# retrojetpacks/Gadget-Leicester

Hardware: AMD Instinct MI355X
Metric: particle-steps/sec (gravity+SPH) (higher is better)
Workload: dtype f64

## Files before the change

### gadget-leicester_amd/csrc/ghip_gravity.hip

```cpp
#include <cmath>

#include "ghip_prim.h"
#include "ghip_walk.h"

__global__ void k_grav_finish(int nt, const int *__restrict__ tgt, const int *__restrict__ perm,
                              int n, double G, double comoving_fac, const double *__restrict__ pos,
                              const double *__restrict__ gravpm, double *__restrict__ oacc,
                              double *__restrict__ oldacc)
{
  int ti = blockIdx.x * blockDim.x + threadIdx.x;
  if(ti >= nt)
    return;
  int i = perm[tgt[ti]];
  double a0 = oacc[i], a1 = oacc[(size_t) n + i], a2 = oacc[2 * (size_t) n + i];
  if(comoving_fac != 0)
    {
      a0 += comoving_fac * pos[i];
      a1 += comoving_fac * pos[(size_t) n + i];
      a2 += comoving_fac * pos[2 * (size_t) n + i];
    }
  double b0 = a0, b1 = a1, b2 = a2;
  if(gravpm)
    {
      b0 = a0 + gravpm[i] / G;
// ... 298 lines not shown
  k_build_segments<<<cdiv(total, 64), 64, 0, ctx->stream>>>(
    ts, P<int4>(t.lk), T, P<int>(t.seg_start), P<int>(t.seg_nanc), P<int>(t.seg_anc));
  HIPCHK(hipGetLastError());
  if(!walk_records)
    return GHIP_OK;
  return ghip_fill_walk_records(ctx, t);
}

int ghip_fill_walk_records(ghip_ctx *ctx, TreeDev &t)
{
  const TreeSizes *ts = P<TreeSizes>(t.dsz);
  const long long ce = (long long) t.n + t.cap_nodes;
  if(ce + 2 >= (1LL << 26))
    return ghip_fail(ctx, GHIP_EINVAL, "the walk addresses its 64-byte element records by a 32-bit byte "
                     "offset: room for %lld elements is more than 2^26", ce);
  GCHK(ghip_ensure(ctx, t.mq, (size_t) (ce + 1) * sizeof(WalkHot)));
  GCHK(ghip_ensure(ctx, t.mq2, (size_t) (ce + 1) * sizeof(WalkCold)));
  k_fill_elems<<<cdiv(ce, 256), 256, 0, ctx->stream>>>(ts, P<double4>(t.xm), P<double4>(t.cl),
                                                      P<int4>(t.lk), P<double>(t.aux),
                                                      P<WalkHot>(t.mq), P<WalkCold>(t.mq2));
  HIPCHK(hipGetLastError());
  return GHIP_OK;
}

int ghip_walk_layout(const TreeDev &t, WalkSeg &sg, int table)
{
  sg.ns = t.seg_ns[table];
  sg.nsub = sg.ns < GHIP_MAXSUB ? sg.ns : GHIP_MAXSUB;
  if(getenv("GHIP_WALK_SUBS"))
    {
      int v = atoi(getenv("GHIP_WALK_SUBS"));
      if(v >= 1 && v <= sg.ns)
        sg.nsub = v;
    }
  if(sg.nsub < 1)
    sg.nsub = 1;
  sg.start = P<int>(t.seg_start) + t.seg_soff[table];
  sg.nanc = P<int>(t.seg_nanc) + t.seg_noff[table];
  sg.anc = P<int>(t.seg_anc) + (size_t) t.seg_noff[table] * GHIP_MAXANC;
  return sg.nsub;
}

static int walk_layout(const TreeDev &t, int nt, WalkSeg &sg, int *nbuckets, bool ewald)
{
  *nbuckets = (nt + 63) / 64;
  static int mid_min = -1;
  if(mid_min < 0)
    {
      mid_min = 3072;
      if(getenv("GHIP_WALK_MID_MIN"))
        mid_min = atoi(getenv("GHIP_WALK_MID_MIN"));
    }
  int table = ewald ? (*nbuckets >= mid_min ? 2 : 1) : (*nbuckets >= mid_min ? 1 : 0);
  return ghip_walk_layout(t, sg, table);
}

struct PartialBufs
{
  double *ax, *ay, *az;
  int *cost;
};

static int ensure_partials(ghip_ctx *ctx, int nwaves, int slot, PartialBufs &pb)
{
  size_t cnt = (size_t) nwaves * 64;
  DevBuf &bx = slot ? ctx->tax2 : ctx->tax, &by = slot ? ctx->tay2 : ctx->tay,
         &bz = slot ? ctx->taz2 : ctx->taz, &bc = slot ? ctx->tcost2 : ctx->tcost;
  GCHK(ghip_ensure(ctx, bx, cnt * 8));
  GCHK(ghip_ensure(ctx, by, cnt * 8));
  GCHK(ghip_ensure(ctx, bz, cnt * 8));
  GCHK(ghip_ensure(ctx, bc, cnt * 4));
  pb.ax = P<double>(bx);
  pb.ay = P<double>(by);
  pb.az = P<double>(bz);
  pb.cost = P<int>(bc);
  return GHIP_OK;
}

static int build_plan(ghip_ctx *ctx, int kind, int nb, int ns, WalkPlan &plan, int slot = 0,
                      hipStream_t on = nullptr)
{
  hipStream_t st = on ? on : ctx->stream;
  DevBuf &b_nsub = slot ? ctx->plan_nsub2 : ctx->plan_nsub, &b_woff = slot ? ctx->plan_woff2 : ctx->plan_woff,
         &b_wave = slot ? ctx->plan_wave2 : ctx->plan_wave;
  int sbase = (49152 + nb - 1) / nb;
  sbase = sbase < 8 ? 8 : (sbase > 64 ? 64 : sbase);
  if(sbase > ns)
    sbase = ns;
  if(getenv("GHIP_WALK_SUBS"))
    {
      int v = atoi(getenv("GHIP_WALK_SUBS"));
      if(v >= 1 && v <= ns)
        sbase = v;
    }
  const int maxwaves = (sbase + 2) * nb + 8;
  GCHK(ghip_ensure(ctx, b_nsub, (size_t) nb * 4));
  GCHK(ghip_ensure(ctx, b_woff, (size_t) (nb + 1) * 4));
  GCHK(ghip_ensure(ctx, b_wave, (size_t) maxwaves * 4));
  int cur = ctx->plan_cur[kind];
  bool prev_kept = ctx->plan_steps[kind][cur].p != nullptr;
  const size_t steps_bytes = ((size_t) nb + nb / 8 + 64) * 4;
  for(int k = 0; k < 2; k++)
    if(ctx->plan_steps[kind][k].cap < (size_t) nb * 4)
      {
        GCHK(ghip_ensure(ctx, ctx->plan_steps[kind][k], steps_bytes));
        if(k == cur)
          prev_kept = false;
      }
  const bool adaptive = !(getenv("GHIP_WALK_ADAPTIVE") && atoi(getenv("GHIP_WALK_ADAPTIVE")) == 0);
  const int pnb = ctx->plan_nb[kind];
  int tol = nb / 16 < 8 ? 8 : nb / 16;
  if(getenv("GHIP_PLAN_EXACT") && atoi(getenv("GHIP_PLAN_EXACT")))
    tol = ctx->plan_ns[kind] == ns ? 0 : -1;
  bool have_prev = adaptive && kind < 2 && pnb > 0 && (pnb > nb ? pnb - nb : nb - pnb) <= tol && prev_kept;
  int nprev = have_prev ? (pnb < nb ? pnb : nb) : 0;
  if(getenv("GHIP_PLAN_DEBUG") && kind < 2)
    {
      static int calls[2], used[2];
      calls[kind]++;
      used[kind] += have_prev;
      if(calls[kind] % 16 == 0)
        fprintf(stderr, "ghip plan kind %d: history used in %d of %d calls (nb %d, before %d)\n", kind,
                used[kind], calls[kind], nb, pnb);
    }
  unsigned int *prev = P<unsigned int>(ctx->plan_steps[kind][cur]);
  unsigned int *out = P<unsigned int>(ctx->plan_steps[kind][cur ^ 1]);
  k_plan_nsub<<<cdiv(nb, 256), 256, 0, st>>>(nb, ns, sbase, prev, nprev, P<int>(b_nsub));
  GCHK(ghip_scan(ctx, P<int>(b_nsub), P<int>(b_woff), nb, st, slot ? &ghip_prim_scratch(ctx, ctx->stream2) : nullptr));
  HIPCHK(hipMemsetAsync(b_wave.p, 0xff, (size_t) maxwaves * 4, st));
  k_plan_fill<<<cdiv(nb, 256), 256, 0, st>>>(nb, P<int>(b_nsub), P<int>(b_woff),
                                             maxwaves, P<int>(b_wave), out,
                                             ghip_errword(ctx, GHIP_ERRW_PLAN));
  HIPCHK(hipGetLastError());
  if(kind < 2)
    {
      ctx->plan_nb[kind] = nb;
      ctx->plan_ns[kind] = ns;
      ctx->plan_cur[kind] = cur ^ 1;
    }
  plan.nwaves = maxwaves;
  plan.wave_bucket = P<int>(b_wave);
  plan.woff = P<int>(b_woff);
  plan.nsub = P<int>(b_nsub);
  plan.steps_out = out;
  plan.started = nullptr;
  plan.started_at = 0;
  return GHIP_OK;
}

template <int MODE>
static void launch_walk(ghip_ctx *ctx, const TreeDev &t, const WalkSeg &sg, int nbuckets, int nt,
                        const int *tgt, const double *tx, const double *ty, const double *tz,
                        const double *tsoft, const double *toldacc, const GravK &k,
                        unsigned long long *counter, const WalkPlan &plan, const PartialBufs &pb,
                        hipStream_t stream)
{
  long long nthreads = (long long) plan.nwaves * 64;
  int bsize = 64;
  if(getenv("GHIP_WALK_BLOCK"))
    {
      int v = atoi(getenv("GHIP_WALK_BLOCK"));
      if(v == 64 || v == 128 || v == 256)
        bsize = v;
    }
  int blocks = cdiv(nthreads, bsize);
  blocks = (blocks + 7) & ~7;
  if(k.xcd_remap > 1)
    blocks = ((blocks + 8 * k.xcd_remap - 1) / (8 * k.xcd_remap)) * (8 * k.xcd_remap);
  WalkPlan pl = plan;
  if(pl.started)
    {
      static double frac = -1;
      if(frac < 0)
        frac = getenv("GHIP_HYDRO_TRIGGER_AT") ? atof(getenv("GHIP_HYDRO_TRIGGER_AT")) : 1.0;
      pl.started_at = (int) (frac * (blocks - 1));
      if(pl.started_at > blocks - 1 || pl.started_at < 0)
        pl.started_at = blocks - 1;
    }
  static int lds_env = -1;
  if(lds_env < 0)
    lds_env = getenv("GHIP_PAIR_NEWTON_LDS") ? atoi(getenv("GHIP_PAIR_NEWTON_LDS")) : 0;
  const int lds_n = lds_env > 0 ? lds_env : ctx->pair_lds;
  static int cap_min = -1;
  if(cap_min < 0)
    cap_min = getenv("GHIP_PAIR_CAP_MIN") ? atoi(getenv("GHIP_PAIR_CAP_MIN")) : 1536;
  static int lds_e = -1;
  if(lds_e < 0)
    lds_e = getenv("GHIP_PAIR_EWALD_LDS") ? atoi(getenv("GHIP_PAIR_EWALD_LDS")) : 0;
  const size_t dyn_lds =
    (MODE == GHIP_WALK_NEWTON && stream != ctx->stream && nbuckets >= cap_min)
      ? (size_t) lds_n
      : ((MODE == GHIP_WALK_EWALD && stream != ctx->stream && nbuckets >= cap_min) ? (size_t) lds_e : 0);
#define GHIP_LAUNCH_WALK(PER, UNEQ)                                                              \
  k_grav_walk<MODE, PER, UNEQ><<<blocks, bsize, dyn_lds, stream>>>(                                \
    t.nelem, P<WalkHot>(t.mq), P<WalkCold>(t.mq2), sg, nt, tgt, tx, ty, tz, tsoft, toldacc, k,     \
    P<float>(ctx->srtab), P<double>((UNEQ) && MODE == GHIP_WALK_EWALD ? ctx->ewbrick : ctx->ewtab),  \
    pb.ax, pb.ay, pb.az, pb.cost, getenv("GHIP_WALK_NOCOUNT") ? nullptr : counter,                  \
    P<unsigned long long>(ctx->rslots) + (counter - P<unsigned long long>(ctx->cslots)), pl)
  static int brick_env = -2;
  if(brick_env == -2)
    brick_env = getenv("GHIP_EW_BRICK") ? atoi(getenv("GHIP_EW_BRICK")) : -1;
  const bool brick = brick_env >= 0 ? brick_env != 0 : true;
  const bool uneq = (MODE == GHIP_WALK_EWALD) ? brick : (bool) k.unequal;
  if(k.periodic && uneq)
    GHIP_LAUNCH_WALK(true, true);
  else if(k.periodic)
    GHIP_LAUNCH_WALK(true, false);
  else if(uneq)
    GHIP_LAUNCH_WALK(false, true);
  else
    GHIP_LAUNCH_WALK(false, false);
#undef GHIP_LAUNCH_WALK
}

static void launch_walk_any(ghip_ctx *ctx, int walk, const TreeDev &t, const WalkSeg &sg,
                            int nbuckets, int nt, const int *tgt, const double *tx,
                            const double *ty, const double *tz, const double *tsoft,
                            const double *toldacc, const GravK &k, unsigned long long *counter,
                            const WalkPlan &plan, const PartialBufs &pb, hipStream_t stream)
{
  if(walk == GHIP_WALK_NEWTON)
    launch_walk<GHIP_WALK_NEWTON>(ctx, t, sg, nbuckets, nt, tgt, tx, ty, tz, tsoft, toldacc, k,
                                  counter, plan, pb, stream);
  else if(walk == GHIP_WALK_SHORTRANGE)
    launch_walk<GHIP_WALK_SHORTRANGE>(ctx, t, sg, nbuckets, nt, tgt, tx, ty, tz, tsoft, toldacc, k,
                                      counter, plan, pb, stream);
  else
    launch_walk<GHIP_WALK_EWALD>(ctx, t, sg, nbuckets, nt, tgt, tx, ty, tz, tsoft, toldacc, k,
                                 counter, plan, pb, stream);
}

static void shard_slice(const ghip_ctx *ctx, int nt, int *lo, int *cnt)
{
  int per;
  ghip_shard_range(nt, ctx->shard_n, ctx->shard_rank, lo, cnt, &per);
}

struct WalkJob
{
  int walk;
  GravK k;
  WalkSeg sg;
  WalkPlan plan;
  PartialBufs pb;
  int nbuckets;
  unsigned long long *counter;
};

static int prepare_job(ghip_ctx *ctx, const ghip_grav_params *p, int walk, int nt, int slot,
                       WalkJob &J, hipStream_t plan_on = nullptr)
{
  hipStream_t ps = plan_on ? plan_on : ctx->stream;
  J.walk = walk;
  GCHK(prepare_tables(ctx, p, walk, J.k));
  walk_layout(ctx->dyn_use ? ctx->dyn.tree : ctx->gt, nt, J.sg, &J.nbuckets, walk == GHIP_WALK_EWALD);
  GCHK(build_plan(ctx, walk == GHIP_WALK_EWALD ? 1 : 0, J.nbuckets, J.sg.ns, J.plan, slot, ps));
  GCHK(ensure_partials(ctx, J.plan.nwaves, slot, J.pb));
  J.counter = ghip_cslot(ctx, walk == GHIP_WALK_EWALD ? GHIP_CK_EWALD : GHIP_CK_NEWTON);
  HIPCHK(hipMemsetAsync(J.counter, 0, GHIP_CKIND_U64 * 8, ps));
  return GHIP_OK;
}

static int run_walk(ghip_ctx *ctx, const WalkJob &J, int nt, const int *tgt, hipStream_t st)
{
  int evi = (J.walk == GHIP_WALK_EWALD) ? 4 : 2;
  ctx->plan_writer[J.walk == GHIP_WALK_EWALD ? 1 : 0] = st;
  HIPCHK(hipEventRecord(ctx->evp[evi], st));
  launch_walk_any(ctx, J.walk, ctx->dyn_use ? ctx->dyn.tree : ctx->gt, J.sg, J.nbuckets, nt, tgt, P<double>(ctx->sx),
                  P<double>(ctx->sy), P<double>(ctx->sz), P<double>(ctx->ssoft),
                  P<double>(ctx->soldacc), J.k, J.counter, J.plan, J.pb, st);
  HIPCHK(hipGetLastError());
  HIPCHK(hipEventRecord(ctx->evp[evi + 1], st));
  return GHIP_OK;
}

static int combine_walk(ghip_ctx *ctx, const WalkJob &J, int nt, const int *tgt, hipStream_t st)
{
  k_combine_grav<<<cdiv(nt, 256), 256, 0, st>>>(
    nt, J.plan, tgt, P<int>(ctx->gt.perm), J.pb.ax, J.pb.ay, J.pb.az, J.pb.cost, ctx->n,
    P<double>(ctx->f[GHIP_F_GRAVACCEL]), P<int>(ctx->f[GHIP_F_GRAVCOST]),
    J.walk == GHIP_WALK_EWALD ? 1 : 0, J.k.debug_steps);
  HIPCHK(hipGetLastError());
  return GHIP_OK;
}

static const int pair_caps[GHIP_PAIR_NSET] = {GHIP_PAIR_LDS(6), GHIP_PAIR_LDS(5), GHIP_PAIR_LDS(4)};

static int pair_setting(int lds)
{
  int k = 0;
  for(int j = 1; j < GHIP_PAIR_NSET; j++)
    if(lds >= pair_caps[j])
      k = j;
  return k;
}

static int pair_balance(ghip_ctx *ctx)
{
  if(!ctx->pc_ev[3][3])
    {
      for(int i = 0; i < 4; i++)
        for(int j = 0; j < 4; j++)
          if(!ctx->pc_ev[i][j])
            HIPCHK(hipEventCreate(&ctx->pc_ev[i][j]));
      return GHIP_OK;
    }
  bool pending[GHIP_PAIR_NSET] = {};
  for(int i = 0; i < 4; i++)
    {
      if(ctx->pc_cap[i] == 0)
        continue;
      hipEvent_t *e = ctx->pc_ev[i];
      if(hipEventQuery(e[1]) != hipSuccess || hipEventQuery(e[3]) != hipSuccess)
        {
          (void) hipGetLastError();
          pending[pair_setting(ctx->pc_cap[i])] = true;
          continue;
        }
      float tn = 0, te = 0;
      if(hipEventElapsedTime(&tn, e[0], e[1]) == hipSuccess && hipEventElapsedTime(&te, e[2], e[3]) == hipSuccess)
        {
          const int k = pair_setting(ctx->pc_cap[i]);
          const float fe = ctx->pc_hyd[i] ? 1.1f : 1.0f;
          const float c = tn > fe * te ? tn : fe * te;
          ctx->pc_cost[k] = c;
          ctx->pc_age[k] = 0;
        }
      else
        (void) hipGetLastError();
      ctx->pc_cap[i] = 0;
    }
  for(int k = 0; k < GHIP_PAIR_NSET; k++)
    ctx->pc_age[k]++;
  const int cur = pair_setting(ctx->pair_lds);
  const float *cost = ctx->pc_cost;
  if(cost[cur] < 0)
    return GHIP_OK;
  int want = cur, probe = -1;
  for(int k = 0; k < GHIP_PAIR_NSET; k++)
// ... 299 lines not shown
```

### gadget-leicester_amd/csrc/ghip_internal.h

```cpp
#pragma once
#include <hip/hip_runtime.h>

#include <cstdint>
#include <cstdio>
#include <cstdlib>
#include <cstring>
#include <new>
#include <string>
#include <vector>

#include "../../include/ghip.h"
#include "ghip_count.h"

#define GHIP_BITS 21
#define GHIP_EN 64
#define GHIP_EW_NB ((GHIP_EN >> 1) + 1)
#define GHIP_EW_NKB (GHIP_EN / 3 + 1)
#define GHIP_EW_DOUBLES (GHIP_EW_NB * GHIP_EW_NB * GHIP_EW_NKB * 16)
static inline __host__ __device__ unsigned int ghip_ew_offset(int i, int j, int kb, int t)
{
  return (unsigned int) ((((i >> 1) * GHIP_EW_NB + (j >> 1)) * GHIP_EW_NKB + kb) * 16 +
                         ((i & 1) * 2 + (j & 1)) * 4 + t);
}
#define GHIP_NTAB 1000
// ... 269 lines not shown
struct PmFft
{
  int n = 0;
  void *fwd = nullptr, *inv = nullptr;
  DevBuf rho, k;
  PmFft() = default;
  PmFft(const PmFft &) = delete;
  PmFft &operator=(const PmFft &) = delete;
  ~PmFft();
};

struct PmMesh
{
  PmFft fft;
  DevBuf force;
  struct Open
  {
    PmFft fft;
    int table_n = 0;
    DevBuf table, force, oct;
  } open;
};

#define GHIP_LDS_PER_CU 163840
#define GHIP_LDS_GRANULE 2048
#define GHIP_PAIR_LDS(W) ((GHIP_LDS_PER_CU / (4 * (W))) / GHIP_LDS_GRANULE * GHIP_LDS_GRANULE)
#define GHIP_PAIR_NSET 3
static_assert(GHIP_PAIR_LDS(4) == 10240 && GHIP_PAIR_LDS(5) == 8192 && GHIP_PAIR_LDS(6) == 6144,
              "dynamic-LDS caps of the pair");

struct ghip_ctx
{
  ghip_ctx() = default;
  ghip_ctx(const ghip_ctx &) = delete;
  ghip_ctx &operator=(const ghip_ctx &) = delete;
  ~ghip_ctx();

  int device = 0;
  hipStream_t stream = nullptr;
  std::string err;

  int n = 0, ngas = 0;
  DevBuf f[GHIP_F_COUNT];
  DevBuf stage, aosP, aosS;
  PinnedWords *pinned = nullptr;

  double corner[3] = {0, 0, 0}, center[3] = {0, 0, 0}, dlen = 0;
  double soft[6] = {0, 0, 0, 0, 0, 0};

  TreeDev gt;
  TreeDev st;
  DevBuf sx, sy, sz, ssoft, soldacc;
  DevBuf gp;
  DevBuf gq;
  DevBuf dleft, dright, drho, dnumngb, ddhsml, ddivv, drot, dflags, dtgt_a, dtgt_b, dhcur;
  DevBuf hpart;

  DevBuf act_host_idx;
  int nactive = -1;
  DevBuf act_next;
  bool gas_mixed = false;
  int skip_massless = 0;
  bool massless_marked = false;
  bool gas_types_unknown = false;
  bool lists_dirty = true;
  bool gas_list_dirty = true;
  DevBuf tg_grav, tg_gas;
  int nt_grav = 0, nt_gas = 0;
  int shard_rank = 0, shard_n = 1;

  DevBuf tax, tay, taz, tcost;
  DevBuf tax2, tay2, taz2, tcost2, plan_nsub2, plan_woff2, plan_wave2, cubtmp2;
  hipStream_t stream2 = nullptr;
  hipStream_t stream3 = nullptr;
  bool adaptive_gravsoft = false;
  bool grav_pending = false;
  unsigned int *pair_started = nullptr;
  bool gas_pending = false;
  bool gas_wait_upload = false;
  hipEvent_t evx[4] = {};
  hipEvent_t evt[2] = {};
  DevBuf plan_steps[3][2], plan_nsub, plan_woff, plan_wave;
  int plan_nb[3] = {-1, -1, -1}, plan_ns[3] = {-1, -1, -1}, plan_cur[3] = {0, 0, 0};
  hipStream_t plan_writer[3] = {nullptr, nullptr, nullptr};
  DevBuf cubtmp3;

  DevBuf ewtab;
  DevBuf ewbrick;
  double ew_box = 0;
  DevBuf srtab;
  bool srtab_ready = false;

  DevBuf cubtmp;
  PmMesh pm;
  ghip_pm_region pm_region = {};
  bool pm_region_set = false;
  DevBuf words;
  DevBuf cslots, rslots;
  ghip_stats stats;
  hipEvent_t ev[16] = {};
  DDState dd;
  DevBuf bh_swallow, bh_injected;
  DevBuf dust_heat;
  DevBuf dust_idx, dust_work, dust_pairs;
  DevBuf sfr_work;
  int timestep_endrun = 0;
  bool iflags_on = false;
  ghip_integration_flags iflags = {};
  DevBuf kick_drag, kick_ddm, kick_newdens;
  bool has_drag = false, has_ddm = false, has_newdens = false;
  int kick_fields_n = -1, kick_fields_ngas = -1;

  bool dust_model_on = false;
  ghip_dust_model dust_model = {};
  bool id_given = false;
  bool visc_on = false;
  ghip_visc_params visc = {};
  DevBuf visc_alpha, visc_dtalpha;
  int visc_ngas = -1;
  long long visc_epoch = 0;

  DevBuf rnd_table;
  int rnd_n = 0;
  unsigned int rnd_gen = 0;

  bool async = false;
  bool tree_unverified = false;
  bool tree_async_ok = true;
  hipEvent_t ev_sizes = nullptr, ev_sizes_gas = nullptr;
  bool gas_unverified = false;
  bool gas_async = false;
  int build_gen = 0;
  bool sort_wide = false;
  bool in_recover = false;
  struct GravCall
  {
    ghip_grav_params p;
    int walk;
  };
  std::vector<GravCall> grav_log;
  std::vector<void *> host_pins;
  bool hydro_early = false;
  bool dyn_on = false, dyn_valid = false, dyn_use = false;
  DynTree dyn;
  int pair_lds = GHIP_PAIR_LDS(5);
  hipEvent_t pc_ev[4][4] = {};
  int pc_cap[4] = {0, 0, 0, 0};
  int pc_hyd[4] = {0, 0, 0, 0};
  int pc_head = 0;
  float pc_cost[GHIP_PAIR_NSET] = {-1.f, -1.f, -1.f};
  int pc_age[GHIP_PAIR_NSET] = {0, 0, 0};
  hipEvent_t ev_side = nullptr;

  std::vector<hipEvent_t> ev_ring;
  int ring_slots = 0, ring_cur = -1;
  hipEvent_t *evp = nullptr;
  long long run_steps = 0, run_syncs0 = 0, run_launches0 = 0, run_dens_iter = 0;
  long long n_syncs = 0;
  DevBuf pot;
  DevBuf pot_nint;
  int pot_n = -1;
  DevBuf potcorr;
  double potcorr_box = 0;
  DevBuf srpot;
  DevBuf gq_work;
};
// ... 225 lines not shown
```

### gadget-leicester_amd/csrc/ghip_walk.h

```cpp
#pragma once
#include "ghip_internal.h"
#include "ghip_count.h"

#ifndef GHIP_WALK_WAVES
#define GHIP_WALK_WAVES 8
#endif
#ifndef GHIP_WALK_OPT
#define GHIP_WALK_OPT 15
#endif


struct GravK
{
  double theta;
  double errtol;
  double boxsize, boxhalf;
  int periodic, unequal;
  int debug_steps;
  int xcd_remap;
  double rcut, rcut2, asmthfac;
  double fac_intp;
  double k1875;
};

// ... 399 lines not shown
          d_skip_to(my_skip, skip);
      next = skip;
      if(open != 0)
        {
          next = e + 1;
          if(skip == next)
            {
              int *w = *(int *volatile *) &d_walk_errw;
              if(w)
                *(volatile int *) w = 1;
            }
        }
    }

  if(OWNED && MODE == GHIP_WALK_NEWTON && (interact & D_BAL(r2 < h2)) == 0)
    {
      const int counted = pidx & 1;
      const int sk = skip;
      if(D_LANE(interact))
        {
          const double fac = (GHIP_WALK_OPT & 8) ? d_mass_over_r3(mass, r2, W.k15, p.k1875)
                                                 : d_mass_over_r3(mass, r2);
          W.acc_x += dx * fac;
          W.acc_y += dy * fac;
          W.acc_z += dz * fac;
          if(GHIP_WALK_OPT & 2)
            W.nint += counted;
          else
            W.nint += (mass > 0) ? 1 : 0;
          if(GHIP_WALK_OPT & 4)
            d_skip_to(my_skip, sk);
        }
      return next;
    }
  if(OWNED && D_LANE(interact))
    {
      if(MODE == GHIP_WALK_EWALD)
        {
          double fx, fy, fz;
          d_ewald_interp<UNEQUAL>(ewtab, p.fac_intp, dx, dy, dz, fx, fy, fz);
          W.acc_x += mass * fx;
          W.acc_y += mass * fy;
          W.acc_z += mass * fz;
          W.nint++;
        }
      else
        {
          double r;
          double fac = d_grav_fac(mass, r2, h, h2, r);
          if(MODE == GHIP_WALK_SHORTRANGE)
            {
              int tabindex = (int) (p.asmthfac * r);
              if(tabindex < GHIP_NTAB)
                {
                  fac *= srtab[tabindex];
                  W.acc_x += dx * fac;
                  W.acc_y += dy * fac;
                  W.acc_z += dz * fac;
                  W.nint++;
                }
            }
          else
            {
              W.acc_x += dx * fac;
              W.acc_y += dy * fac;
              W.acc_z += dz * fac;
              if(mass > 0)
                W.nint++;
            }
        }
    }
  return next;
}

struct WalkPlan
{
  int nwaves;
  const int *__restrict__ wave_bucket;
  const int *__restrict__ woff;
  const int *__restrict__ nsub;
  unsigned int *__restrict__ steps_out;
  unsigned int *started;
  int started_at;
};

struct SegCursor
{
  int kseg;
  int e, s1;
};

template <int MODE, bool PERIODIC, bool UNEQUAL, bool REL>
__device__ __forceinline__ bool d_enter_segment(SegCursor &c, int stride, const WalkSeg &sg,
                                                const WalkHot *__restrict__ hot,
                                                const WalkCold *__restrict__ cold, const GravK &p,
                                                const float *__restrict__ srtab,
                                                const double *__restrict__ ewtab, bool valid,
                                                WalkLane &W, int &my_skip, unsigned int &steps)
{
  while(c.kseg < sg.ns)
    {
      const int s0 = __builtin_amdgcn_readfirstlane(sg.start[c.kseg]);
      c.s1 = __builtin_amdgcn_readfirstlane(sg.start[c.kseg + 1]);
      my_skip = valid ? 0 : 0x7fffffff;
      const int na = __builtin_amdgcn_readfirstlane(sg.nanc[c.kseg]);
      for(int a = 0; a < na; a++)
        {
          int ea = __builtin_amdgcn_readfirstlane(sg.anc[c.kseg * GHIP_MAXANC + a]);
          v16i H;
          d_load1(hot, ea, H);
          d_walk_element<MODE, PERIODIC, UNEQUAL, false, REL>(ea, H, cold, p, srtab, ewtab, W, my_skip);
          steps++;
        }
      int first = d_wave_min_i32(my_skip);
      c.e = __builtin_amdgcn_readfirstlane(first > s0 ? first : s0);
      if(c.e < c.s1)
        return true;
      c.kseg += stride;
    }
  return false;
}

template <int MODE, bool PERIODIC, bool UNEQUAL, bool REL>
__device__ __forceinline__ void d_walk_run(const WalkSeg &sg, int sub, const WalkHot *__restrict__ hot,
                                           const WalkCold *__restrict__ cold, const GravK &p,
                                           const float *__restrict__ srtab,
                                           const double *__restrict__ ewtab, bool valid, WalkLane &W,
                                           unsigned int &steps)
{
  if(MODE != GHIP_WALK_EWALD)
    {
      SegCursor A;
      int skipA = 0;
      A.kseg = sub;
      const int stride = sg.nsub;
      bool liveA = d_enter_segment<MODE, PERIODIC, UNEQUAL, REL>(A, stride, sg, hot, cold, p, srtab,
                                                            ewtab, valid, W, skipA, steps);
      int t1 = 0, t2 = 0;
      while(liveA)
        {
          v16i HA;
          const unsigned int offA = d_rec_off(A.e);
          d_load1_touch(hot, offA, HA, t1, t2);
          d_touch_next(hot, offA, t1);
          d_touch(hot, d_lo32(HA, 6), t2);
          steps++;
          A.e = __builtin_amdgcn_readfirstlane(
            d_walk_element<MODE, PERIODIC, UNEQUAL, true, REL>(A.e, HA, cold, p, srtab, ewtab, W, skipA));
          if(__builtin_expect(A.e >= A.s1, 0))
            {
              d_drain_touch(t1, t2);
              A.kseg += stride;
              liveA = d_enter_segment<MODE, PERIODIC, UNEQUAL, REL>(A, stride, sg, hot, cold, p, srtab,
                                                               ewtab, valid, W, skipA, steps);
            }
        }
      d_drain_touch(t1, t2);
    }
  else
    {
      SegCursor A, B;
      int skipA = 0, skipB = 0;
      A.kseg = sub;
      B.kseg = sub + sg.nsub;
      const int stride = 2 * sg.nsub;
      bool liveA = d_enter_segment<MODE, PERIODIC, UNEQUAL, REL>(A, stride, sg, hot, cold, p, srtab, ewtab, valid,
                                                   W, skipA, steps);
      bool liveB = d_enter_segment<MODE, PERIODIC, UNEQUAL, REL>(B, stride, sg, hot, cold, p, srtab, ewtab, valid,
                                                   W, skipB, steps);
      while(liveA && liveB)
        {
          v16i HA, HB;
          d_load2(hot, A.e, HA, B.e, HB);
          steps += 2;
          A.e = __builtin_amdgcn_readfirstlane(
            d_walk_element<MODE, PERIODIC, UNEQUAL, true, REL>(A.e, HA, cold, p, srtab, ewtab, W, skipA));
          B.e = __builtin_amdgcn_readfirstlane(
            d_walk_element<MODE, PERIODIC, UNEQUAL, true, REL>(B.e, HB, cold, p, srtab, ewtab, W, skipB));
          if(A.e >= A.s1)
            {
              A.kseg += stride;
              liveA = d_enter_segment<MODE, PERIODIC, UNEQUAL, REL>(A, stride, sg, hot, cold, p, srtab, ewtab,
                                                      valid, W, skipA, steps);
            }
          if(B.e >= B.s1)
            {
              B.kseg += stride;
              liveB = d_enter_segment<MODE, PERIODIC, UNEQUAL, REL>(B, stride, sg, hot, cold, p, srtab, ewtab,
                                                      valid, W, skipB, steps);
            }
        }
      if(liveB)
        {
          A = B;
          skipA = skipB;
          liveA = true;
        }
      while(liveA)
        {
          v16i HA;
          d_load1(hot, A.e, HA);
          steps++;
          A.e = __builtin_amdgcn_readfirstlane(
            d_walk_element<MODE, PERIODIC, UNEQUAL, true, REL>(A.e, HA, cold, p, srtab, ewtab, W, skipA));
          if(A.e >= A.s1)
            {
              A.kseg += stride;
              liveA = d_enter_segment<MODE, PERIODIC, UNEQUAL, REL>(A, stride, sg, hot, cold, p, srtab, ewtab,
                                                      valid, W, skipA, steps);
            }
        }
    }

}

template <int MODE, bool PERIODIC, bool UNEQUAL>
__global__ void __launch_bounds__(GHIP_BLOCK) __attribute__((amdgpu_waves_per_eu(MODE == GHIP_WALK_EWALD ? 4 : GHIP_WALK_WAVES, 8)))
k_grav_walk(int nelem, const WalkHot *__restrict__ hot, const WalkCold *__restrict__ cold,
            WalkSeg sg, int nt, const int *__restrict__ tgt, const double *__restrict__ tx,
            const double *__restrict__ ty, const double *__restrict__ tz,
            const double *__restrict__ tsoft, const double *__restrict__ toldacc, GravK p,
            const float *__restrict__ srtab, const double *__restrict__ ewtab,
            double *__restrict__ pax, double *__restrict__ pay, double *__restrict__ paz,
            int *__restrict__ pcost, unsigned long long *__restrict__ counter,
            unsigned long long *__restrict__ acc, WalkPlan plan)
{
  const int lane = threadIdx.x & 63;
  if(plan.started && blockIdx.x == plan.started_at && threadIdx.x == 0)
    __hip_atomic_store(plan.started, 1u, __ATOMIC_RELEASE, __HIP_MEMORY_SCOPE_SYSTEM);
  const int per_xcd = gridDim.x >> 3;
  int lblock = blockIdx.x;
  if(p.xcd_remap == 1)
    lblock = (blockIdx.x & 7) * per_xcd + (blockIdx.x >> 3);
  else if(p.xcd_remap > 1)
    {
      const int j = blockIdx.x >> 3, x = blockIdx.x & 7, G = p.xcd_remap;
      lblock = ((j / G) * 8 + x) * G + (j % G);
    }
  const int wave = __builtin_amdgcn_readfirstlane((lblock * (int) blockDim.x + threadIdx.x) >> 6);
  if(wave >= plan.nwaves)
    return;
  const int bucket = __builtin_amdgcn_readfirstlane(plan.wave_bucket[wave]);
  if(bucket < 0 || bucket * 64 >= nt)
    return;
  const int sub = wave - __builtin_amdgcn_readfirstlane(plan.woff[bucket]);
  sg.nsub = __builtin_amdgcn_readfirstlane(plan.nsub[bucket]);
  const int ti = bucket * 64 + lane;
  const bool valid = ti < nt;
  const int s = valid ? (tgt ? tgt[ti] : ti) : 0;

  WalkLane W;
  W.pos_x = W.pos_y = W.pos_z = 0;
  W.h_i = 1;
  W.aold = 0;
  W.h2 = 1;
  if(valid)
    {
      W.pos_x = tx[s];
      W.pos_y = ty[s];
      W.pos_z = tz[s];
      W.h_i = tsoft[s];
      W.aold = p.errtol * toldacc[s];
      W.h2 = W.h_i * W.h_i;
    }
  W.acc_x = W.acc_y = W.acc_z = 0;
  W.nint = 0;
  W.k15 = 1.5;
  asm volatile("" : "+v"(W.k15));
  unsigned int steps = 0;

  if(p.theta == 0)
    d_walk_run<MODE, PERIODIC, UNEQUAL, true>(sg, sub, hot, cold, p, srtab, ewtab, valid, W, steps);
  else
    d_walk_run<MODE, PERIODIC, UNEQUAL, false>(sg, sub, hot, cold, p, srtab, ewtab, valid, W, steps);

  if(valid)
    {
      const size_t o = (size_t) wave * 64 + lane;
      pax[o] = W.acc_x;
      pay[o] = W.acc_y;
      paz[o] = W.acc_z;
      pcost[o] = p.debug_steps ? (int) steps : W.nint;
    }
  unsigned long long tot = d_wave_sum_u64((unsigned long long) W.nint);
  if(lane == 0 && tot && counter)
    {
      d_count(counter, 0, tot);
      d_count(acc, 0, tot);
    }
  if(lane == 0)
    {
      if(counter)
        {
          d_count(counter, 1, (unsigned long long) steps);
          d_count(acc, 1, (unsigned long long) steps);
        }
      atomicAdd(plan.steps_out + bucket, steps);
    }
}

__global__ void k_plan_nsub(int nb, int ns, int sbase, const unsigned int *__restrict__ steps_prev,
                            int nprev, int *__restrict__ nsub)
{
  __shared__ unsigned long long part[4];
  unsigned long long tot = 0;
  if(nprev > 0)
    {
      for(int k = threadIdx.x; k < nprev; k += blockDim.x)
        tot += steps_prev[k];
      for(int o = 32; o > 0; o >>= 1)
        tot += __shfl_xor(tot, o);
      if((threadIdx.x & 63) == 0)
        part[threadIdx.x >> 6] = tot;
      __syncthreads();
      tot = part[0] + part[1] + part[2] + part[3];
    }
  int b = blockIdx.x * blockDim.x + threadIdx.x;
  if(b >= nb)
    return;
  int s = ns < sbase ? ns : sbase;
  if(b < nprev && tot > 0)
    {
      double mean = (double) tot / (double) nprev;
      s = (int) ((double) sbase * (double) steps_prev[b] / mean) + 1;
      s = s < 2 ? 2 : s;
      s = s > 64 ? 64 : s;
      if(s > ns)
        s = ns;
    }
  nsub[b] = s < 1 ? 1 : s;
}

__global__ void k_plan_fill(int nb, const int *__restrict__ nsub, const int *__restrict__ woff,
                            int maxwaves, int *__restrict__ wave_bucket,
                            unsigned int *__restrict__ steps_out, int *__restrict__ errword)
{
  int b = blockIdx.x * blockDim.x + threadIdx.x;
  if(b >= nb)
    return;
  int o = woff[b], s = nsub[b];
  if(o + s > maxwaves)
    *(volatile int *) errword = 1;
  for(int q = 0; q < s; q++)
    if(o + q < maxwaves)
      wave_bucket[o + q] = b;
  steps_out[b] = 0;
}

struct SegTables
{
  int ntab;
  int ns[3], soff[3], noff[3];
};

__global__ void k_build_segments(const TreeSizes *__restrict__ ts, const int4 *__restrict__ lk,
                                 SegTables T, int *__restrict__ start, int *__restrict__ nanc,
                                 int *__restrict__ anc)
{
  const int nelem = ts->nelem;
  int g = blockIdx.x * blockDim.x + threadIdx.x;
  int j = 0;
  while(j < T.ntab && g > T.ns[j])
    {
      g -= T.ns[j] + 1;
      j++;
    }
  if(j >= T.ntab)
    return;
  const int ns = T.ns[j], k = g;
  start += T.soff[j];
  nanc += T.noff[j];
  anc += (size_t) T.noff[j] * GHIP_MAXANC;
  long long chunk = ((long long) nelem + ns - 1) / ns;
  long long s0l = (long long) k * chunk;
  int s0 = (int) (s0l > nelem ? nelem : s0l);
  if(k == ns)
    s0 = nelem;
  start[k] = s0;
  if(k == ns)
    return;
  int na = 0, e = 0;
  while(e < s0)
    {
      int4 q = lk[e];
      if(!LK_IS_PARTICLE(q) && q.x > s0)
        {
          if(na < GHIP_MAXANC)
            anc[k * GHIP_MAXANC + na] = e;
          na++;
          e = e + 1;
        }
      else
        e = q.x;
    }
  nanc[k] = na < GHIP_MAXANC ? na : GHIP_MAXANC;
}

__global__ void k_combine_grav(int nt, WalkPlan plan, const int *__restrict__ tgt,
                               const int *__restrict__ perm, const double *__restrict__ pax,
                               const double *__restrict__ pay, const double *__restrict__ paz,
                               const int *__restrict__ pcost, int n, double *__restrict__ oacc,
                               int *__restrict__ ocost, int accumulate, int debug_max)
{
  int ti = blockIdx.x * blockDim.x + threadIdx.x;
  if(ti >= nt)
    return;
  const int bucket = ti >> 6, lane = ti & 63;
  const int w0 = plan.woff[bucket];
  int nsub = plan.nsub[bucket];
  if(w0 + nsub > plan.nwaves)
    nsub = plan.nwaves > w0 ? plan.nwaves - w0 : 0;
  double a0 = 0, a1 = 0, a2 = 0;
  int c = 0;
  for(int s = 0; s < nsub; s++)
    {
      size_t o = (size_t) (w0 + s) * 64 + lane;
      a0 += pax[o];
      a1 += pay[o];
      a2 += paz[o];
      c = debug_max ? (pcost[o] > c ? pcost[o] : c) : c + pcost[o];
    }
  int i = perm ? perm[tgt[ti]] : ti;
  if(accumulate)
    {
      oacc[i] += a0;
      oacc[(size_t) n + i] += a1;
      oacc[2 * (size_t) n + i] += a2;
      ocost[i] += c;
    }
// ... 98 lines not shown
```

Baseline: 84.49 million.

## Assign contiguous cost-balanced segment runs to walk waves using per-segment cost history

Replaces the strided segment-to-wave assignment in the gravity tree walk with contiguous runs of segments per wave. The run boundaries come from a new planning kernel that splits per-bucket segment costs recorded in the previous step into equal-cost pieces, with a midpoint split for the two interleaved cursors. The walk kernel now records per-segment step costs for the next plan. The aim is to balance work across the sub-waves of each bucket and improve locality, at the cost of an extra planning kernel, per-segment cost stores, and larger history buffers.

```diff
diff --git a/gadget-leicester_amd/csrc/ghip_gravity.hip b/gadget-leicester_amd/csrc/ghip_gravity.hip
--- a/gadget-leicester_amd/csrc/ghip_gravity.hip
+++ b/gadget-leicester_amd/csrc/ghip_gravity.hip
@@ -404,7 +404,10 @@
 {
   hipStream_t st = on ? on : ctx->stream;
   DevBuf &b_nsub = slot ? ctx->plan_nsub2 : ctx->plan_nsub, &b_woff = slot ? ctx->plan_woff2 : ctx->plan_woff,
-         &b_wave = slot ? ctx->plan_wave2 : ctx->plan_wave;
+         &b_wave = slot ? ctx->plan_wave2 : ctx->plan_wave, &b_seg = slot ? ctx->plan_seg2 : ctx->plan_seg;
+  static int runs = -1;
+  if(runs < 0)
+    runs = !(getenv("GHIP_WALK_RUNS") && atoi(getenv("GHIP_WALK_RUNS")) == 0);
   int sbase = (49152 + nb - 1) / nb;
   sbase = sbase < 8 ? 8 : (sbase > 64 ? 64 : sbase);
   if(sbase > ns)
@@ -429,6 +432,21 @@
         if(k == cur)
           prev_kept = false;
       }
+  bool seg_kept = false;
+  if(runs && kind < 2)
+    {
+      seg_kept = ctx->plan_segcost[kind][cur].p != nullptr;
+      const size_t seg_bytes = ((size_t) nb + nb / 8 + 64) * ns * 4;
+      for(int k = 0; k < 2; k++)
+        if(ctx->plan_segcost[kind][k].cap < (size_t) nb * ns * 4)
+          {
+            GCHK(ghip_ensure(ctx, ctx->plan_segcost[kind][k], seg_bytes));
+            if(k == cur)
+              seg_kept = false;
+          }
+    }
+  if(runs)
+    GCHK(ghip_ensure(ctx, b_seg, ((size_t) maxwaves + 1) * 4));
   const bool adaptive = !(getenv("GHIP_WALK_ADAPTIVE") && atoi(getenv("GHIP_WALK_ADAPTIVE")) == 0);
   const int pnb = ctx->plan_nb[kind];
   int tol = nb / 16 < 8 ? 8 : nb / 16;
@@ -436,14 +454,20 @@
     tol = ctx->plan_ns[kind] == ns ? 0 : -1;
   bool have_prev = adaptive && kind < 2 && pnb > 0 && (pnb > nb ? pnb - nb : nb - pnb) <= tol && prev_kept;
   int nprev = have_prev ? (pnb < nb ? pnb : nb) : 0;
+  const bool have_seg = have_prev && seg_kept && ctx->plan_ns[kind] == ns;
   if(getenv("GHIP_PLAN_DEBUG") && kind < 2)
     {
-      static int calls[2], used[2];
+      static int calls[2], used[2], used_seg[2];
       calls[kind]++;
       used[kind] += have_prev;
+      used_seg[kind] += have_seg;
       if(calls[kind] % 16 == 0)
         fprintf(stderr, "ghip plan kind %d: history used in %d of %d calls (nb %d, before %d)\n", kind,
                 used[kind], calls[kind], nb, pnb);
+      if(atoi(getenv("GHIP_PLAN_DEBUG")) >= 2)
+        fprintf(stderr, "ghip plan kind %d call %d: runs %d nb %d (before %d) ns %d (before %d) bucket_history %d "
+                "segment_history %d (used in %d calls)\n", kind, calls[kind], runs, nb, pnb, ns, ctx->plan_ns[kind],
+                (int) have_prev, (int) have_seg, used_seg[kind]);
     }
   unsigned int *prev = P<unsigned int>(ctx->plan_steps[kind][cur]);
   unsigned int *out = P<unsigned int>(ctx->plan_steps[kind][cur ^ 1]);
@@ -453,6 +477,13 @@
   k_plan_fill<<<cdiv(nb, 256), 256, 0, st>>>(nb, P<int>(b_nsub), P<int>(b_woff),
                                              maxwaves, P<int>(b_wave), out,
                                              ghip_errword(ctx, GHIP_ERRW_PLAN));
+  if(runs)
+    {
+      const int wg = ghip_wg(ctx);
+      k_plan_runs<<<cdiv(nb, wg), wg, 0, st>>>(nb, ns, P<int>(b_nsub), P<int>(b_woff), maxwaves,
+                                               have_seg ? P<unsigned int>(ctx->plan_segcost[kind][cur]) : nullptr,
+                                               have_seg ? nprev : 0, P<unsigned int>(b_seg));
+    }
   HIPCHK(hipGetLastError());
   if(kind < 2)
     {
@@ -467,6 +498,8 @@
   plan.steps_out = out;
   plan.started = nullptr;
   plan.started_at = 0;
+  plan.wave_seg = runs ? P<unsigned int>(b_seg) : nullptr;
+  plan.seg_cost = runs && kind < 2 ? P<unsigned int>(ctx->plan_segcost[kind][cur ^ 1]) : nullptr;
   return GHIP_OK;
 }
 
@@ -513,12 +546,21 @@
     (MODE == GHIP_WALK_NEWTON && stream != ctx->stream && nbuckets >= cap_min)
       ? (size_t) lds_n
       : ((MODE == GHIP_WALK_EWALD && stream != ctx->stream && nbuckets >= cap_min) ? (size_t) lds_e : 0);
-#define GHIP_LAUNCH_WALK(PER, UNEQ)                                                              \
-  k_grav_walk<MODE, PER, UNEQ><<<blocks, bsize, dyn_lds, stream>>>(                                \
+#define GHIP_LAUNCH_WALK_R(PER, UNEQ, RUNS)                                                      \
+  k_grav_walk<MODE, PER, UNEQ, RUNS><<<blocks, bsize, dyn_lds, stream>>>(                          \
     t.nelem, P<WalkHot>(t.mq), P<WalkCold>(t.mq2), sg, nt, tgt, tx, ty, tz, tsoft, toldacc, k,     \
     P<float>(ctx->srtab), P<double>((UNEQ) && MODE == GHIP_WALK_EWALD ? ctx->ewbrick : ctx->ewtab),  \
     pb.ax, pb.ay, pb.az, pb.cost, getenv("GHIP_WALK_NOCOUNT") ? nullptr : counter,                  \
     P<unsigned long long>(ctx->rslots) + (counter - P<unsigned long long>(ctx->cslots)), pl)
+#define GHIP_LAUNCH_WALK(PER, UNEQ)                                                              \
+  do                                                                                             \
+    {                                                                                            \
+      if(pl.wave_seg)                                                                            \
+        GHIP_LAUNCH_WALK_R(PER, UNEQ, true);                                                     \
+      else                                                                                       \
+        GHIP_LAUNCH_WALK_R(PER, UNEQ, false);                                                    \
+    }                                                                                            \
+  while(0)
   static int brick_env = -2;
   if(brick_env == -2)
     brick_env = getenv("GHIP_EW_BRICK") ? atoi(getenv("GHIP_EW_BRICK")) : -1;
@@ -533,6 +575,7 @@
   else
     GHIP_LAUNCH_WALK(false, false);
 #undef GHIP_LAUNCH_WALK
+#undef GHIP_LAUNCH_WALK_R
 }
 
 static void launch_walk_any(ghip_ctx *ctx, int walk, const TreeDev &t, const WalkSeg &sg,
@@ -577,6 +620,21 @@
   GCHK(prepare_tables(ctx, p, walk, J.k));
   walk_layout(ctx->dyn_use ? ctx->dyn.tree : ctx->gt, nt, J.sg, &J.nbuckets, walk == GHIP_WALK_EWALD);
   GCHK(build_plan(ctx, walk == GHIP_WALK_EWALD ? 1 : 0, J.nbuckets, J.sg.ns, J.plan, slot, ps));
+  if(getenv("GHIP_PLAN_DEBUG") && atoi(getenv("GHIP_PLAN_DEBUG")) >= 3)
+    {
+      static int calls[2];
+      const int kind = walk == GHIP_WALK_EWALD ? 1 : 0;
+      if(calls[kind]++ % 16 == 0)
+        {
+          std::vector<int> na(J.sg.ns);
+          HIPCHK(ghip_stream_sync(ctx, ctx->stream));
+          HIPCHK(hipMemcpy(na.data(), J.sg.nanc, (size_t) J.sg.ns * 4, hipMemcpyDeviceToHost));
+          double sum = 0;
+          for(int v : na)
+            sum += v;
+          fprintf(stderr, "ghip plan kind %d: %d segments, mean ancestor count %.2f\n", kind, J.sg.ns, sum / J.sg.ns);
+        }
+    }
   GCHK(ensure_partials(ctx, J.plan.nwaves, slot, J.pb));
   J.counter = ghip_cslot(ctx, walk == GHIP_WALK_EWALD ? GHIP_CK_EWALD : GHIP_CK_NEWTON);
   HIPCHK(hipMemsetAsync(J.counter, 0, GHIP_CKIND_U64 * 8, ps));
diff --git a/gadget-leicester_amd/csrc/ghip_internal.h b/gadget-leicester_amd/csrc/ghip_internal.h
--- a/gadget-leicester_amd/csrc/ghip_internal.h
+++ b/gadget-leicester_amd/csrc/ghip_internal.h
@@ -375,6 +375,7 @@
   hipEvent_t evt[2] = {};
   DevBuf plan_steps[3][2], plan_nsub, plan_woff, plan_wave;
   int plan_nb[3] = {-1, -1, -1}, plan_ns[3] = {-1, -1, -1}, plan_cur[3] = {0, 0, 0};
+  DevBuf plan_segcost[2][2], plan_seg, plan_seg2;
   hipStream_t plan_writer[3] = {nullptr, nullptr, nullptr};
   DevBuf cubtmp3;
 
diff --git a/gadget-leicester_amd/csrc/ghip_walk.h b/gadget-leicester_amd/csrc/ghip_walk.h
--- a/gadget-leicester_amd/csrc/ghip_walk.h
+++ b/gadget-leicester_amd/csrc/ghip_walk.h
@@ -505,24 +505,54 @@
   unsigned int *__restrict__ steps_out;
   unsigned int *started;
   int started_at;
+  const unsigned int *__restrict__ wave_seg;
+  unsigned int *__restrict__ seg_cost;
 };
 
 struct SegCursor
 {
   int kseg;
   int e, s1;
+  int end;
+  int stride;
+  unsigned int mark;
 };
 
-template <int MODE, bool PERIODIC, bool UNEQUAL, bool REL>
-__device__ __forceinline__ bool d_enter_segment(SegCursor &c, int stride, const WalkSeg &sg,
+__device__ __forceinline__ void d_put_cost(unsigned int *__restrict__ cost, int k, unsigned int v)
+{
+  if(cost && __lane_id() == 0)
+    cost[k] = v;
+}
+
+template <int MODE>
+__device__ __forceinline__ bool d_next_segment(SegCursor &c, const WalkSeg &sg,
+                                               unsigned int *__restrict__ cost, unsigned int steps)
+{
+  for(;;)
+    {
+      d_put_cost(cost, c.kseg, MODE == GHIP_WALK_EWALD ? c.mark : steps - c.mark);
+      c.mark = MODE == GHIP_WALK_EWALD ? 0u : steps;
+      c.kseg++;
+      if(c.kseg >= c.end)
+        return false;
+      c.s1 = __builtin_amdgcn_readfirstlane(sg.start[c.kseg + 1]);
+      if(c.e < c.s1)
+        return true;
+    }
+}
+
+template <int MODE, bool PERIODIC, bool UNEQUAL, bool REL, bool RUNS>
+__device__ __forceinline__ bool d_enter_segment(SegCursor &c, const WalkSeg &sg,
                                                 const WalkHot *__restrict__ hot,
                                                 const WalkCold *__restrict__ cold, const GravK &p,
                                                 const float *__restrict__ srtab,
                                                 const double *__restrict__ ewtab, bool valid,
-                                                WalkLane &W, int &my_skip, unsigned int &steps)
-{
-  while(c.kseg < sg.ns)
-    {
+                                                WalkLane &W, int &my_skip, unsigned int &steps,
+                                                unsigned int *__restrict__ cost)
+{
+  while(c.kseg < c.end)
+    {
+      const unsigned int before = steps;
       const int s0 = __builtin_amdgcn_readfirstlane(sg.start[c.kseg]);
       c.s1 = __builtin_amdgcn_readfirstlane(sg.start[c.kseg + 1]);
       my_skip = valid ? 0 : 0x7fffffff;
@@ -537,15 +567,37 @@
         }
       int first = d_wave_min_i32(my_skip);
       c.e = __builtin_amdgcn_readfirstlane(first > s0 ? first : s0);
+      if(RUNS)
+        {
+          c.mark = MODE == GHIP_WALK_EWALD ? steps - before : before;
+          return c.e < c.s1 ? true : d_next_segment<MODE>(c, sg, cost, steps);
+        }
       if(c.e < c.s1)
         return true;
-      c.kseg += stride;
+      c.kseg += c.stride;
     }
   return false;
 }
 
-template <int MODE, bool PERIODIC, bool UNEQUAL, bool REL>
-__device__ __forceinline__ void d_walk_run(const WalkSeg &sg, int sub, const WalkHot *__restrict__ hot,
+template <int MODE, bool PERIODIC, bool UNEQUAL, bool REL, bool RUNS>
+__device__ __forceinline__ bool d_switch_segment(SegCursor &c, const WalkSeg &sg,
+                                                 const WalkHot *__restrict__ hot,
+                                                 const WalkCold *__restrict__ cold, const GravK &p,
+                                                 const float *__restrict__ srtab,
+                                                 const double *__restrict__ ewtab, bool valid,
+                                                 WalkLane &W, int &my_skip, unsigned int &steps,
+                                                 unsigned int *__restrict__ cost)
+{
+  if(RUNS)
+    return d_next_segment<MODE>(c, sg, cost, steps);
+  c.kseg += c.stride;
+  return d_enter_segment<MODE, PERIODIC, UNEQUAL, REL, false>(c, sg, hot, cold, p, srtab, ewtab, valid, W,
+                                                              my_skip, steps, cost);
+}
+
+template <int MODE, bool PERIODIC, bool UNEQUAL, bool REL, bool RUNS>
+__device__ __forceinline__ void d_walk_run(const WalkSeg &sg, int lo, int mid, int hi, int stride,
+                                           unsigned int *__restrict__ cost, const WalkHot *__restrict__ hot,
                                            const WalkCold *__restrict__ cold, const GravK &p,
                                            const float *__restrict__ srtab,
                                            const double *__restrict__ ewtab, bool valid, WalkLane &W,
@@ -555,10 +607,12 @@
     {
       SegCursor A;
       int skipA = 0;
-      A.kseg = sub;
-      const int stride = sg.nsub;
-      bool liveA = d_enter_segment<MODE, PERIODIC, UNEQUAL, REL>(A, stride, sg, hot, cold, p, srtab,
-                                                            ewtab, valid, W, skipA, steps);
+      A.kseg = lo;
+      A.end = hi;
+      A.stride = stride;
+      A.mark = 0;
+      bool liveA = d_enter_segment<MODE, PERIODIC, UNEQUAL, REL, RUNS>(A, sg, hot, cold, p, srtab, ewtab,
+                                                                  valid, W, skipA, steps, cost);
       int t1 = 0, t2 = 0;
       while(liveA)
         {
@@ -573,9 +627,8 @@
           if(__builtin_expect(A.e >= A.s1, 0))
             {
               d_drain_touch(t1, t2);
-              A.kseg += stride;
-              liveA = d_enter_segment<MODE, PERIODIC, UNEQUAL, REL>(A, stride, sg, hot, cold, p, srtab,
-                                                               ewtab, valid, W, skipA, steps);
+              liveA = d_switch_segment<MODE, PERIODIC, UNEQUAL, REL, RUNS>(A, sg, hot, cold, p, srtab, ewtab,
+                                                                      valid, W, skipA, steps, cost);
             }
         }
       d_drain_touch(t1, t2);
@@ -584,34 +637,33 @@
     {
       SegCursor A, B;
       int skipA = 0, skipB = 0;
-      A.kseg = sub;
-      B.kseg = sub + sg.nsub;
-      const int stride = 2 * sg.nsub;
-      bool liveA = d_enter_segment<MODE, PERIODIC, UNEQUAL, REL>(A, stride, sg, hot, cold, p, srtab, ewtab, valid,
-                                                   W, skipA, steps);
-      bool liveB = d_enter_segment<MODE, PERIODIC, UNEQUAL, REL>(B, stride, sg, hot, cold, p, srtab, ewtab, valid,
-                                                   W, skipB, steps);
+      A.kseg = lo;
+      A.end = RUNS ? mid : hi;
+      B.kseg = RUNS ? mid : lo + stride;
+      B.end = hi;
+      A.stride = B.stride = 2 * stride;
+      A.mark = B.mark = 0;
+      bool liveA = d_enter_segment<MODE, PERIODIC, UNEQUAL, REL, RUNS>(A, sg, hot, cold, p, srtab, ewtab, valid,
+                                                         W, skipA, steps, cost);
+      bool liveB = d_enter_segment<MODE, PERIODIC, UNEQUAL, REL, RUNS>(B, sg, hot, cold, p, srtab, ewtab, valid,
+                                                         W, skipB, steps, cost);
       while(liveA && liveB)
         {
           v16i HA, HB;
           d_load2(hot, A.e, HA, B.e, HB);
           steps += 2;
+          A.mark++;
+          B.mark++;
           A.e = __builtin_amdgcn_readfirstlane(
             d_walk_element<MODE, PERIODIC, UNEQUAL, true, REL>(A.e, HA, cold, p, srtab, ewtab, W, skipA));
           B.e = __builtin_amdgcn_readfirstlane(
             d_walk_element<MODE, PERIODIC, UNEQUAL, true, REL>(B.e, HB, cold, p, srtab, ewtab, W, skipB));
           if(A.e >= A.s1)
-            {
-              A.kseg += stride;
-              liveA = d_enter_segment<MODE, PERIODIC, UNEQUAL, REL>(A, stride, sg, hot, cold, p, srtab, ewtab,
-                                                      valid, W, skipA, steps);
-            }
+            liveA = d_switch_segment<MODE, PERIODIC, UNEQUAL, REL, RUNS>(A, sg, hot, cold, p, srtab, ewtab, valid,
+                                                               W, skipA, steps, cost);
           if(B.e >= B.s1)
-            {
-              B.kseg += stride;
-              liveB = d_enter_segment<MODE, PERIODIC, UNEQUAL, REL>(B, stride, sg, hot, cold, p, srtab, ewtab,
-                                                      valid, W, skipB, steps);
-            }
+            liveB = d_switch_segment<MODE, PERIODIC, UNEQUAL, REL, RUNS>(B, sg, hot, cold, p, srtab, ewtab, valid,
+                                                               W, skipB, steps, cost);
         }
       if(liveB)
         {
@@ -624,20 +676,18 @@
           v16i HA;
           d_load1(hot, A.e, HA);
           steps++;
+          A.mark++;
           A.e = __builtin_amdgcn_readfirstlane(
             d_walk_element<MODE, PERIODIC, UNEQUAL, true, REL>(A.e, HA, cold, p, srtab, ewtab, W, skipA));
           if(A.e >= A.s1)
-            {
-              A.kseg += stride;
-              liveA = d_enter_segment<MODE, PERIODIC, UNEQUAL, REL>(A, stride, sg, hot, cold, p, srtab, ewtab,
-                                                      valid, W, skipA, steps);
-            }
-        }
-    }
-
-}
-
-template <int MODE, bool PERIODIC, bool UNEQUAL>
+            liveA = d_switch_segment<MODE, PERIODIC, UNEQUAL, REL, RUNS>(A, sg, hot, cold, p, srtab, ewtab, valid,
+                                                               W, skipA, steps, cost);
+        }
+    }
+
+}
+
+template <int MODE, bool PERIODIC, bool UNEQUAL, bool RUNS>
 __global__ void __launch_bounds__(GHIP_BLOCK) __attribute__((amdgpu_waves_per_eu(MODE == GHIP_WALK_EWALD ? 4 : GHIP_WALK_WAVES, 8)))
 k_grav_walk(int nelem, const WalkHot *__restrict__ hot, const WalkCold *__restrict__ cold,
             WalkSeg sg, int nt, const int *__restrict__ tgt, const double *__restrict__ tx,
@@ -668,6 +718,19 @@
     return;
   const int sub = wave - __builtin_amdgcn_readfirstlane(plan.woff[bucket]);
   sg.nsub = __builtin_amdgcn_readfirstlane(plan.nsub[bucket]);
+  int seg_lo = sub, seg_mid = sub, seg_hi = sg.ns;
+  const int seg_stride = sg.nsub;
+  if(RUNS)
+    {
+      const unsigned int w0 = __builtin_amdgcn_readfirstlane(plan.wave_seg[wave]);
+      seg_hi = sub + 1 < sg.nsub ? (int) (__builtin_amdgcn_readfirstlane(plan.wave_seg[wave + 1]) & 0xffffu) : sg.ns;
+      seg_hi = seg_hi < sg.ns ? seg_hi : sg.ns;
+      seg_lo = (int) (w0 & 0xffffu);
+      seg_lo = seg_lo < seg_hi ? seg_lo : seg_hi;
+      seg_mid = (int) (w0 >> 16);
+      seg_mid = seg_mid < seg_lo ? seg_lo : (seg_mid > seg_hi ? seg_hi : seg_mid);
+    }
+  unsigned int *__restrict__ seg_cost = RUNS && plan.seg_cost ? plan.seg_cost + (size_t) bucket * sg.ns : nullptr;
   const int ti = bucket * 64 + lane;
   const bool valid = ti < nt;
   const int s = valid ? (tgt ? tgt[ti] : ti) : 0;
@@ -693,9 +756,11 @@
   unsigned int steps = 0;
 
   if(p.theta == 0)
-    d_walk_run<MODE, PERIODIC, UNEQUAL, true>(sg, sub, hot, cold, p, srtab, ewtab, valid, W, steps);
+    d_walk_run<MODE, PERIODIC, UNEQUAL, true, RUNS>(sg, seg_lo, seg_mid, seg_hi, seg_stride, seg_cost, hot, cold, p,
+                                              srtab, ewtab, valid, W, steps);
   else
-    d_walk_run<MODE, PERIODIC, UNEQUAL, false>(sg, sub, hot, cold, p, srtab, ewtab, valid, W, steps);
+    d_walk_run<MODE, PERIODIC, UNEQUAL, false, RUNS>(sg, seg_lo, seg_mid, seg_hi, seg_stride, seg_cost, hot, cold, p,
+                                               srtab, ewtab, valid, W, steps);
 
   if(valid)
     {
@@ -768,6 +833,53 @@
     if(o + q < maxwaves)
       wave_bucket[o + q] = b;
   steps_out[b] = 0;
+}
+
+__global__ void k_plan_runs(int nb, int ns, const int *__restrict__ nsub, const int *__restrict__ woff,
+                            int maxwaves, const unsigned int *__restrict__ cost_prev, int nprev,
+                            unsigned int *__restrict__ wave_seg)
+{
+  const int b = blockIdx.x * blockDim.x + threadIdx.x;
+  if(b >= nb)
+    return;
+  const int S = nsub[b], o = woff[b];
+  const unsigned int *c = b < nprev ? cost_prev + (size_t) b * ns : nullptr;
+  unsigned long long total = 0;
+  if(c)
+    for(int k = 0; k < ns; k++)
+      total += c[k];
+  const unsigned long long M = 2ull * (unsigned long long) S;
+  int k = 0;
+  unsigned long long P = 0;
+  int c0 = 0, c1 = 0;
+  for(int j = 0; j <= 2 * S; j++)
+    {
+      int cut;
+      if(j == 2 * S)
+        cut = ns;
+      else if(total == 0)
+        cut = (int) ((long long) j * ns / (2 * S));
+      else
+        {
+          const unsigned long long want = (unsigned long long) j * total;
+          while(k < ns && P * M < want)
+            P += c[k++];
+          cut = k;
+          if(k > 0 && P * M > want && want - (P - c[k - 1]) * M < P * M - want)
+            cut = k - 1;
+        }
+      if(j >= 2 && (j & 1) == 0)
+        {
+          const int q = j / 2 - 1;
+          int mid = c1;
+          if(cut - c0 >= 2)
+            mid = mid <= c0 ? c0 + 1 : (mid >= cut ? cut - 1 : mid);
+          if(o + q < maxwaves)
+            wave_seg[o + q] = (unsigned int) c0 | ((unsigned int) mid << 16);
+        }
+      c0 = c1;
+      c1 = cut;
+    }
 }
 
 struct SegTables
```

Measured after the change: 83.66 million. About the same (-1.0%).
